# caburu/gym-supplychain

Hardware: AMD Instinct MI355X
Metric: env-steps/sec at 65536 envs/GPU, beergame-v0; 1/2/4/8 MI355X (higher is better)
Workload: dtype int32; 1 GPU; beergame-v0 step() x 65536 envs/GPU (BASELINE configs[1]; configs[4] at N=8); n_envs_per_gpu=65536, levels=4, weeks=35, auto_reset=True, ledgers=True, orders_history=True, episode_return_allgather=False, parallelism=env-shard x1

## Files before the change

### gym-supplychain_amd/csrc/scg_beergame.hip

```cpp

#include <cstdarg>
#include <cstdio>
#include <ctime>
#include <vector>

#include "scg_beergame_kernels.h"

namespace scg {

__global__ __launch_bounds__(kBlock) void poisson_demand_kernel(const BgArgs a, int32_t weeks,
                                                                int32_t* __restrict__ out) {
  const int64_t n = static_cast<int64_t>(blockIdx.x) * kBlock + threadIdx.x;
  if (n >= a.n) return;
  for (int32_t w = 1; w <= weeks; ++w) out[(int64_t)(w - 1) * a.n + n] = week_demand(a, n, w, a.episode);
}

__global__ __launch_bounds__(kBlock) void uniform_ints_kernel(uint32_t k0, uint32_t k1, int64_t env_offset,
                                                              int64_t n_envs, int32_t rows, int32_t width,
                                                              uint32_t tag, int32_t lo, uint32_t range,
                                                              int32_t* __restrict__ out) {
  const int64_t n = static_cast<int64_t>(blockIdx.x) * kBlock + threadIdx.x;
  if (n >= n_envs) return;
  const uint32_t env = static_cast<uint32_t>(env_offset + n);
  const int32_t words = rows * width;
  for (int32_t j0 = 0; j0 < words; j0 += 4) {
    const scg::U4 r = scg::philox4x32_10(scg::U4{env, tag, static_cast<uint32_t>(j0 >> 2), SCG_STREAM_ACTION}, k0, k1);
    const uint32_t w4[4] = {r.x, r.y, r.z, r.w};
#pragma unroll
    for (int s = 0; s < 4; ++s) {
      const int32_t j = j0 + s;
      if (j < words) {
        const uint32_t v = static_cast<uint32_t>((static_cast<uint64_t>(w4[s]) * range) >> 32);
        const int32_t rrow = j / width, col = j - rrow * width;
        out[((int64_t)rrow * n_envs + n) * width + col] = lo + static_cast<int32_t>(v);
      }
    }
  }
}

int launch_reset(int L, dim3 grid, hipStream_t s, const BgArgs& a) {
  switch (L) {
#define X(l) case l: return bg_launch_reset<l>(grid, s, a);
    SCG_LEVEL_CASES(X)
#undef X
    default: return fail(SCG_ERR_INVALID, "levels=%d outside 1..%d", L, SCG_BG_MAX_LEVELS);
  }
}

int launch_step2(int L, dim3 grid, hipStream_t s, const BgArgs& a, const WeekInfo& wk) {
  switch (L) {
#define X(l) case l: return bg_launch_step2<l>(grid, s, a, wk);
    SCG_LEVEL_CASES(X)
#undef X
    default: return fail(SCG_ERR_INVALID, "levels=%d outside 1..%d", L, SCG_BG_MAX_LEVELS);
  }
}

int launch_step(int L, dim3 grid, hipStream_t s, const BgArgs& a, const WeekInfo& wk, hipEvent_t ev0,
                hipEvent_t ev1) {
  switch (L) {
#define X(l) case l: return bg_launch_step<l>(grid, s, a, wk, ev0, ev1);
    SCG_LEVEL_CASES(X)
#undef X
    default: return fail(SCG_ERR_INVALID, "levels=%d outside 1..%d", L, SCG_BG_MAX_LEVELS);
  }
}

int launch_server(int L, int demand_mode, hipStream_t s, scg_bg_server_box* box, uint32_t exit_seen,
                  uint32_t idle_ticks) {
  switch (L) {
#define X(l) case l: return bg_launch_server<l>(s, demand_mode, box, exit_seen, idle_ticks);
    SCG_LEVEL_CASES(X)
#undef X
    default: return fail(SCG_ERR_INVALID, "levels=%d outside 1..%d", L, SCG_BG_MAX_LEVELS);
  }
}

int launch_slab(int demand_mode, int L, dim3 grid, hipStream_t s, int32_t* slab, const int32_t* act, int32_t* out,
                uint32_t n32, uint32_t wpack, uint32_t week, uint32_t episode, uint32_t k0, uint32_t k1,
                const BgSlabArgs& a, hipEvent_t ev0, hipEvent_t ev1) {
  switch (L) {
#define X(l) case l: return bg_launch_slab<l>(demand_mode, grid, s, slab, act, out, n32, wpack, week, episode, k0, k1, a, ev0, ev1);
    SCG_LEVEL_CASES(X)
#undef X
    default: return fail(SCG_ERR_INVALID, "levels=%d outside 1..%d", L, SCG_BG_MAX_LEVELS);
  }
}

int launch_rollout(int L, dim3 grid, hipStream_t s, const BgArgs& a, int32_t K, const RolloutWeeks& weeks,
                   const int32_t* acts, int32_t* obs, int32_t* rew) {
  switch (L) {
#define X(l) case l: return bg_launch_rollout<l>(grid, s, a, K, weeks, acts, obs, rew);
    SCG_LEVEL_CASES(X)
#undef X
    default: return fail(SCG_ERR_INVALID, "levels=%d outside 1..%d", L, SCG_BG_MAX_LEVELS);
  }
}

int slab_layout(int L, int64_t N, int32_t R, int32_t T, bool history, int64_t* off) {
  const int64_t NL = N * L;
  if (NL % 4 != 0) return fail(SCG_ERR_INVALID, "slab layout needs n_envs * levels %% 4 == 0 (got %lld)", (long long)NL);
  if (R < 1 || R > 127) return fail(SCG_ERR_INVALID, "slab layout needs 1 <= ring_slots <= 127");
  off[SCG_SLAB_ERROR] = 0;
  for (int f = 0; f < 6; ++f) off[SCG_SLAB_INVENTORY + f] = kSlabHeader + f * NL;
  off[SCG_SLAB_RING] = kSlabHeader + 6 * NL;
  off[SCG_SLAB_EPISODE_RETURN] = kSlabHeader + (6 + R) * NL;
  off[SCG_SLAB_FINAL_RETURN] = off[SCG_SLAB_EPISODE_RETURN] + 2 * N;
  off[SCG_SLAB_HISTORY] = off[SCG_SLAB_FINAL_RETURN] + 2 * N;
  off[SCG_SLAB_TOTAL] = off[SCG_SLAB_HISTORY] + (history ? static_cast<int64_t>(T + 1) * NL : 0);
  return SCG_OK;
}

bool slab_ready(const scg_bg_config* cfg, const scg_bg_state* st, const int32_t* obs, const int32_t* reward,
                const int32_t* terminal_obs) {
  if (!st->slab || cfg->variant != 1) return false;
  int64_t off[SCG_SLAB_FIELDS];
  const bool hist = st->orders_history != nullptr;
  if (slab_layout(cfg->levels, st->n_envs, cfg->ring_slots, cfg->max_weeks, hist, off) != SCG_OK) return false;
  int32_t* b = st->slab;
  const bool ledgers = st->inventory_costs != nullptr, returns = st->episode_return != nullptr;
  return st->inventory == b + off[SCG_SLAB_INVENTORY] && st->backlog == b + off[SCG_SLAB_BACKLOG] &&
         st->orders_placed == b + off[SCG_SLAB_ORDERS] && st->shipments == b + off[SCG_SLAB_RING] &&
         (!ledgers || (st->inventory_costs == b + off[SCG_SLAB_INV_COSTS] &&
                       st->backlog_costs == b + off[SCG_SLAB_BACKLOG_COSTS])) &&
         ledgers == (st->backlog_costs != nullptr) &&
         (!returns || (reinterpret_cast<int32_t*>(st->episode_return) == b + off[SCG_SLAB_EPISODE_RETURN] &&
                       reinterpret_cast<int32_t*>(st->final_return) == b + off[SCG_SLAB_FINAL_RETURN])) &&
         (!hist || st->orders_history == b + off[SCG_SLAB_HISTORY]) &&
         st->error_flags == b + off[SCG_SLAB_ERROR] && reward == obs + st->n_envs * cfg->levels &&
         (!terminal_obs || terminal_obs == b + off[SCG_SLAB_TERMINAL_OBS]);
}

int check_state(const scg_bg_config* cfg, const scg_bg_state* st) {
  if (!cfg || !st) return fail(SCG_ERR_INVALID, "null config/state");
  if (!cfg->plan || cfg->ring_slots <= 0) return fail(SCG_ERR_INVALID, "config not prepared (call scg_bg_prepare)");
  if (st->n_envs <= 0) return fail(SCG_ERR_INVALID, "n_envs must be > 0");
  if (st->n_envs > INT32_MAX) return fail(SCG_ERR_INVALID, "n_envs must be <= %d per shard", INT32_MAX);
  if (st->env_offset < 0 || st->env_offset + st->n_envs > (int64_t(1) << 32))
    return fail(SCG_ERR_INVALID, "global env ids must fit in 32 bits");
  if (!st->inventory || !st->backlog || !st->orders_placed || !st->shipments)
    return fail(SCG_ERR_INVALID, "state buffers inventory/backlog/orders_placed/shipments are required");
  if (cfg->demand_mode == SCG_DEMAND_TABLE && !cfg->demand_table)
    return fail(SCG_ERR_INVALID, "TABLE demand mode needs demand_table");
  if (cfg->demand_mode == SCG_DEMAND_POISSON && !cfg->poisson_thresholds)
    return fail(SCG_ERR_INVALID, "POISSON demand mode needs poisson_thresholds");
  return SCG_OK;
}

inline int32_t init_slots(const scg_bg_config* cfg) {
  const int32_t d0 = cfg->shipment_delays ? cfg->shipment_delays[0] : 0;
  return cfg->full_table ? d0 : std::min(d0, cfg->max_weeks);
}

BgArgs make_args(const scg_bg_config* cfg, const scg_bg_state* st) {
  BgArgs a;
  std::memset(&a, 0, sizeof(a));
  a.inv = st->inventory;
  a.bk = st->backlog;
  a.op = st->orders_placed;
  a.ring = st->shipments;
  a.inv_acc = st->inventory_costs;
  a.bk_acc = st->backlog_costs;
  a.hist = st->orders_history;
  a.ep_ret = st->episode_return;
  a.final_ret = st->final_return;
// ... 96 lines not shown
    if (cfg->variant != 1) return fail(SCG_ERR_INVALID, "full_table is a BeerGameEnv (variant 1) option");
    int32_t last = T + 1;
    for (int32_t w = 0; w <= T; ++w) last = std::max(last, w + cfg->shipment_delays[w] + 1);
    R = last + 1;
  }
  std::vector<uint8_t> written(static_cast<size_t>(T) + SCG_BG_MAX_DELAY + 2, 0);
  for (int32_t t = 1; t <= init_slots(cfg); ++t) written[t] = 1;
  cfg->plan[0] = 0;
  for (int32_t w = 1; w <= T; ++w) {
    const int32_t d = cfg->shipment_delays[w];
    int32_t mode;
    if (d == 0) {
      mode = MODE_DIRECT;
    } else if (w + d > T && !full) {
      mode = MODE_DROP;
    } else if (written[w + d]) {
      mode = MODE_ADD;
    } else {
      mode = MODE_STORE;
      written[w + d] = 1;
    }
    cfg->plan[w] = mode | (written[w] ? PLAN_ARRIVE : 0) | (d << 8);
  }
  cfg->ring_slots = R;
  return SCG_OK;
}

int scg_bg_slab_layout(const scg_bg_config* cfg, int64_t n_envs, int32_t with_history,
                       int64_t offsets[SCG_SLAB_FIELDS]) {
  if (!cfg || !offsets) return fail(SCG_ERR_INVALID, "null config/offsets");
  if (cfg->ring_slots <= 0) return fail(SCG_ERR_INVALID, "config not prepared (call scg_bg_prepare)");
  if (n_envs <= 0 || n_envs > INT32_MAX) return fail(SCG_ERR_INVALID, "n_envs must be in 1..%d", INT32_MAX);
  return slab_layout(cfg->levels, n_envs, cfg->ring_slots, cfg->max_weeks, with_history != 0, offsets);
}

int scg_bg_reset(const scg_bg_config* cfg, scg_bg_state* st, int32_t* obs, void* stream) {
  if (int rc = check_state(cfg, st)) return rc;
  if (st->week >= 0) st->episode += 1;
  BgArgs a = make_args(cfg, st);
  a.obs = obs;
  if (int rc = launch_reset(cfg->levels, grid_for(st->n_envs), static_cast<hipStream_t>(stream), a)) return rc;
  st->week = 0;
  return SCG_OK;
}

static scg::WeekInfo week_info(const scg_bg_config* cfg, int32_t w, uint32_t flags) {
  const int32_t p = cfg->plan[w];
  const int32_t R = cfg->ring_slots;
  WeekInfo wk;
  wk.week = w;
  wk.read_slot = plan_arrive(p) ? w % R : -1;
  wk.write_slot = (w + plan_delay(p)) % R;
  wk.mode = plan_mode(p);
  wk.demand_fixed = cfg->demand_mode == SCG_DEMAND_FIXED ? cfg->customer_demand[w - 1] : 0;
  const bool terminal = (w == cfg->max_weeks);
  wk.flags = (terminal ? 1 : 0) | ((terminal && (flags & SCG_BG_AUTORESET)) ? 2 : 0);
  return wk;
}

static int check_step(const scg_bg_config* cfg, const scg_bg_state* st) {
  if (st->week < 0) return fail(SCG_ERR_NOT_RESET, "step() before reset()");
  if (st->week >= cfg->max_weeks)
    return fail(SCG_ERR_PAST_HORIZON, "step() after the terminal week %d (customer_demand has %d weeks)",
                cfg->max_weeks, cfg->max_weeks);
  return SCG_OK;
}

int scg_bg_step(const scg_bg_config* cfg, scg_bg_state* st, const int32_t* action, int32_t* obs,
                int32_t* reward, int32_t* terminal_obs, uint32_t flags, int32_t* done, void* stream) {
  return scg_bg_step_timed(cfg, st, action, obs, reward, terminal_obs, flags, done, nullptr, nullptr, stream);
}

int scg_bg_step_timed(const scg_bg_config* cfg, scg_bg_state* st, const int32_t* action, int32_t* obs,
                      int32_t* reward, int32_t* terminal_obs, uint32_t flags, int32_t* done, void* start_event,
                      void* stop_event, void* stream) {
  if (int rc = check_state(cfg, st)) return rc;
  if (!action || !obs || !reward) return fail(SCG_ERR_INVALID, "action/obs/reward buffers are required");
  if (int rc = check_step(cfg, st)) return rc;
  const int32_t w = st->week + 1;
  const WeekInfo wk = week_info(cfg, w, flags);
  if (slab_ready(cfg, st, obs, reward, terminal_obs)) {
    BgSlabArgs sa;
    std::memset(&sa, 0, sizeof(sa));
    sa.pthr = cfg->poisson_thresholds;
    sa.demand_table = cfg->demand_table;
    sa.pthr_len = cfg->poisson_len;
    sa.h = cfg->inv_cost;
    sa.b = cfg->backlog_cost;
    sa.demand_fixed = wk.demand_fixed;
    sa.demand_lo = cfg->demand_lo;
    sa.demand_hi = cfg->demand_hi;
    sa.ship_value = cfg->initial_shipment_value;
    sa.orders_value = cfg->initial_orders_value;
    sa.init_slots = init_slots(cfg);
    sa.env_offset = st->env_offset;
    sa.guard = week_guard(cfg->levels, cfg->inv_cost, cfg->backlog_cost);
    sa.err_host = st->error_host;
    for (int l = 0; l < cfg->levels; ++l) sa.init_inv[l] = cfg->initial_inventory[l];
    uint32_t wpack = pack_week_slab(wk);
    wpack |= (wk.flags & 1) ? SW_TERMINAL : 0u;
    wpack |= (wk.flags & 2) ? SW_AUTORESET : 0u;
    wpack |= st->inventory_costs ? SW_LEDGERS : 0u;
    wpack |= st->episode_return ? SW_RETURNS : 0u;
    wpack |= st->orders_history ? SW_HISTORY : 0u;
    wpack |= static_cast<uint32_t>(cfg->ring_slots) << 24;
    if (int rc = launch_slab(cfg->demand_mode, cfg->levels, grid_for(st->n_envs), static_cast<hipStream_t>(stream),
                             st->slab, action, obs, static_cast<uint32_t>(st->n_envs), wpack, static_cast<uint32_t>(w),
                             st->episode, static_cast<uint32_t>(st->seed & 0xffffffffu),
                             static_cast<uint32_t>(st->seed >> 32), sa, static_cast<hipEvent_t>(start_event),
                             static_cast<hipEvent_t>(stop_event)))
      return rc;
    if (wk.flags & 2) {
      st->week = 0;
      st->episode += 1;
    } else {
      st->week = w;
    }
    if (done) *done = (wk.flags & 1) ? 1 : 0;
    return SCG_OK;
  }
  BgArgs a = make_args(cfg, st);
  a.act = action;
  a.obs = obs;
  a.rew = reward;
  a.term_obs = terminal_obs;
  if (cfg->variant == 2) {
    if (int rc = launch_step2(cfg->levels, grid_for(st->n_envs), static_cast<hipStream_t>(stream), a, wk)) return rc;
  } else if (int rc = launch_step(cfg->levels, grid_for(st->n_envs), static_cast<hipStream_t>(stream), a, wk,
                                  static_cast<hipEvent_t>(start_event), static_cast<hipEvent_t>(stop_event))) {
    return rc;
  }
  if (wk.flags & 2) {
    st->week = 0;
    st->episode += 1;
  } else {
    st->week = w;
  }
  if (done) *done = (wk.flags & 1) ? 1 : 0;
  return SCG_OK;
}

static_assert(sizeof(scg_bg_server_line) == 64, "request line");
static_assert(sizeof(scg_bg_server_box) == 17 * 64 + 64 + SCG_BG_SERVER_SLOTS * SCG_BG_SERVER_ARGS_BYTES, "mailbox");
static_assert(offsetof(scg_bg_server_box, done_seq) == 16 * 64 && offsetof(scg_bg_server_box, args) == 18 * 64,
              "mailbox lines");
static_assert(sizeof(scg_bg_server) == 72 && sizeof(scg_bg_server_slot) == 64, "server structs");
struct ServerLock {
  int32_t* w;
  explicit ServerLock(scg_bg_server* sv) : w(&sv->lock) {
    for (;;) {
      int32_t z = 0;
      if (__atomic_compare_exchange_n(w, &z, 1, false, __ATOMIC_ACQUIRE, __ATOMIC_RELAXED)) return;
      cpu_relax();
    }
  }
  ~ServerLock() { __atomic_store_n(w, 0, __ATOMIC_RELEASE); }
};

static bool server_ok(const scg_bg_server* sv) { return sv && sv->box_host && sv->box_dev; }

static int server_launch_locked(scg_bg_server* sv) {
  const uint32_t exit_seen = __atomic_load_n(&sv->box_host->exit_req, __ATOMIC_ACQUIRE);
  const uint32_t idle_ticks = static_cast<uint32_t>(sv->idle_us) * 100u;
  if (int rc = launch_server(sv->levels, sv->demand_mode, static_cast<hipStream_t>(sv->stream), sv->box_dev,
                             exit_seen, idle_ticks))
    return rc;
  sv->running = 1;
  sv->launches += 1;
  sv->last_ns = mono_ns();
  return SCG_OK;
}

static int server_stop_locked(scg_bg_server* sv) {
  if (!sv->running) return SCG_OK;
  __atomic_store_n(&sv->box_host->exit_req, sv->box_host->exit_req + 1, __ATOMIC_RELEASE);
  sv->running = 0;
  if (hipStreamSynchronize(static_cast<hipStream_t>(sv->stream)) != hipSuccess)
    return fail(SCG_ERR_HIP, "step server: hipStreamSynchronize failed");
  return SCG_OK;
}

int scg_bg_server_stop(scg_bg_server* sv) {
  if (!server_ok(sv)) return fail(SCG_ERR_INVALID, "null server/mailbox");
  ServerLock lk(sv);
  return server_stop_locked(sv);
}

uint32_t scg_bg_server_line_check(const scg_bg_server_line* line) {
  uint32_t w[16];
  std::memcpy(w, line, sizeof(w));
  return server_line_check(w);
}

// ... 212 lines not shown
```

### gym-supplychain_amd/csrc/scg_beergame_kernels.h

```cpp
#pragma once

#include <hip/hip_ext.h>
#include <hip/hip_runtime.h>

#include <algorithm>
#include <cmath>
#include <cstdint>
#include <cstdlib>
#include <cstring>

#include "scg_common.h"
#include "scg_mailbox.h"
#include "scg_const.h"
#include "scg_philox.h"
#include "scgpu.h"

namespace scg {

enum : int32_t { MODE_DIRECT = 0, MODE_STORE = 1, MODE_ADD = 2, MODE_DROP = 3 };
constexpr int32_t PLAN_ARRIVE = 4;
inline int32_t plan_mode(int32_t p) { return p & 3; }
inline bool plan_arrive(int32_t p) { return (p & PLAN_ARRIVE) != 0; }
inline int32_t plan_delay(int32_t p) { return (p >> 8) & 0xff; }

constexpr int kBlock = 256;

struct BgArgs {
  int32_t* inv;
  int32_t* bk;
  int32_t* op;
  int32_t* ring;
  int32_t* inv_acc;
  int32_t* bk_acc;
  int32_t* hist;
  int64_t* ep_ret;
  int64_t* final_ret;
  const int32_t* act;
  int32_t* obs;
  int32_t* rew;
  int32_t* term_obs;
  const int32_t* demand_table;
  const uint32_t* pthr;
  int64_t n;
  int64_t env_offset;
  uint32_t key0, key1;
  uint32_t episode;
  int32_t demand_mode;
  int32_t pthr_len;
  int32_t h, b;
  int32_t ship_value, orders_value;
  int32_t init_slots;
  int32_t ring_slots;
  int32_t init_inv[SCG_BG_MAX_LEVELS];
  int32_t* pen_acc;
  int32_t max_stock, penalty;
  int32_t demand_lo, demand_hi;
  int32_t stochastic_delays, delay_lo, delay_hi, max_weeks;
  int32_t* err;
  int32_t guard;
  int32_t* err_host;
};

#ifndef SCG_BG_OVERFLOW_CHECK
#define SCG_BG_OVERFLOW_CHECK 1
#endif
__device__ __forceinline__ bool fits32(int64_t x) {
  return !SCG_BG_OVERFLOW_CHECK || x == static_cast<int64_t>(static_cast<int32_t>(x));
}
__device__ __forceinline__ int out32(int64_t x) { return fits32(x) ? 0 : 1; }

__device__ __forceinline__ void note_overflow(int32_t* err, bool ovf) {
  if (ovf && err) *reinterpret_cast<volatile int32_t*>(err) = 1;
}

__device__ __forceinline__ void export_error(int64_t n, bool terminal, const int32_t* err, int32_t* err_host) {
  if (terminal && n == 0 && err && err_host)
    *reinterpret_cast<volatile int32_t*>(err_host) = *reinterpret_cast<const volatile int32_t*>(err);
}

template <int L>
__device__ __forceinline__ void load_row(const int32_t* __restrict__ p, int32_t (&v)[L]) {
  if constexpr (L % 4 == 0) {
#pragma unroll
    for (int c = 0; c < L / 4; ++c) {
      const int4 t = reinterpret_cast<const int4*>(p)[c];
      v[4 * c] = t.x; v[4 * c + 1] = t.y; v[4 * c + 2] = t.z; v[4 * c + 3] = t.w;
    }
  } else if constexpr (L % 2 == 0) {
#pragma unroll
// ... 386 lines not shown
static_assert(sizeof(BgArgs) <= SCG_BG_SERVER_ARGS_BYTES, "BgArgs outgrew the mailbox's argument blocks");
static_assert(kServerSlots <= 16 && kServerArgWords <= 2 * kServerBlock, "server layout");

template <int L, int DM>
__global__ __launch_bounds__(kServerBlock) void bg_server_kernel(scg_bg_server_box* box, uint32_t exit_seen,
                                                                 uint32_t idle_ticks) {
  __shared__ __align__(16) uint32_t s_args[kServerSlots][kServerArgWords];
  __shared__ uint32_t s_last[16], s_gen[16];
  const int lane = threadIdx.x;
  if (lane < 16) {
    s_last[lane] = __hip_atomic_load(&box->done_seq[lane], __ATOMIC_RELAXED, __HIP_MEMORY_SCOPE_SYSTEM);
    s_gen[lane] = 0;
  }
  __syncthreads();
  const uint32_t* lines = reinterpret_cast<const uint32_t*>(box->req);
  uint64_t t0 = __builtin_amdgcn_s_memrealtime();
  uint32_t ex = exit_seen;
  uint32_t ns = __hip_atomic_load(&box->n_slots, __ATOMIC_RELAXED, __HIP_MEMORY_SCOPE_SYSTEM);
  for (;;) {
    const int n_slots = __builtin_amdgcn_readfirstlane(static_cast<int>(ns < kServerSlots ? ns : kServerSlots));
    ns = __hip_atomic_load(&box->n_slots, __ATOMIC_RELAXED, __HIP_MEMORY_SCOPE_SYSTEM);
    ex = __hip_atomic_load(&box->exit_req, __ATOMIC_RELAXED, __HIP_MEMORY_SCOPE_SYSTEM);
    uint32_t v[4] = {0, 0, 0, 0};
#pragma unroll
    for (int r = 0; r < 4; ++r) {
      const int slot = 4 * r + (lane >> 4);
      if (slot < n_slots)
        v[r] = __hip_atomic_load(lines + slot * 16 + (lane & 15), __ATOMIC_RELAXED, __HIP_MEMORY_SCOPE_SYSTEM);
    }
    bool served = false;
    for (int slot = 0; slot < n_slots; ++slot) {
      const int base = (slot & 3) * 16, r = slot >> 2;
      const uint32_t vr = r == 0 ? v[0] : r == 1 ? v[1] : r == 2 ? v[2] : v[3];
      const uint32_t seq = __builtin_amdgcn_readlane(vr, base);
      if (seq == s_last[slot]) continue;
      uint32_t w[16];
#pragma unroll
      for (int i = 0; i < 16; ++i) w[i] = __builtin_amdgcn_readlane(vr, base + i);
      if (w[7] != server_line_check(w)) continue;
      __builtin_amdgcn_fence(__ATOMIC_ACQUIRE, "");
      if (w[6] != s_gen[slot]) {
        const uint32_t* src = reinterpret_cast<const uint32_t*>(box->args[slot]);
        for (int k = lane; k < kServerArgWords; k += kServerBlock)
          s_args[slot][k] = __hip_atomic_load(src + k, __ATOMIC_RELAXED, __HIP_MEMORY_SCOPE_SYSTEM);
        __syncthreads();
        if (lane == 0) s_gen[slot] = w[6];
      }
      const BgArgs& a = *reinterpret_cast<const BgArgs*>(s_args[slot]);
      WeekInfo wk{};
      wk.week = static_cast<int32_t>(w[3]);
      wk.demand_fixed = static_cast<int32_t>(w[4]);
      const int64_t n = lane;
      if (n < a.n) {
        if (L <= 8 && static_cast<int32_t>(w[5]) == L) {
          int32_t act_in[L];
#pragma unroll
          for (int l = 0; l < L; ++l) act_in[l] = static_cast<int32_t>(w[8 + (l < 8 ? l : 0)]);
          bg_step_env<L, DM, true>(n, a.inv, a.bk, a.op, a.act, a.ring, static_cast<uint32_t>(a.n), w[2], a, wk, act_in);
        } else {
          bg_step_env<L, DM>(n, a.inv, a.bk, a.op, a.act, a.ring, static_cast<uint32_t>(a.n), w[2], a, wk);
        }
      }
      __builtin_amdgcn_fence(__ATOMIC_RELEASE, "");
      if (lane == 0) {
        __hip_atomic_store(&box->done_seq[slot], seq, __ATOMIC_RELEASE, __HIP_MEMORY_SCOPE_SYSTEM);
        s_last[slot] = seq;
      }
      __syncthreads();
      served = true;
    }
    if (ex != exit_seen) break;
    if (served) {
      t0 = __builtin_amdgcn_s_memrealtime();
      continue;
    }
    if (__builtin_amdgcn_s_memrealtime() - t0 > idle_ticks) break;
    __builtin_amdgcn_s_sleep(2);
  }
  __builtin_amdgcn_fence(__ATOMIC_RELEASE, "");
  if (lane == 0) __hip_atomic_store(&box->exit_seq, ex, __ATOMIC_RELEASE, __HIP_MEMORY_SCOPE_SYSTEM);
}

struct BgSlabArgs {
  const uint32_t* pthr;
  const int32_t* demand_table;
  int32_t pthr_len;
  int32_t h, b;
  int32_t demand_fixed;
  int32_t demand_lo, demand_hi;
  int32_t ship_value, orders_value, init_slots;
  int64_t env_offset;
  int32_t guard;
  int32_t* err_host;
  int32_t init_inv[SCG_BG_MAX_LEVELS];
};


constexpr uint32_t SW_TERMINAL = 1u << 18, SW_AUTORESET = 1u << 19, SW_LEDGERS = 1u << 20, SW_RETURNS = 1u << 21,
                   SW_HISTORY = 1u << 22;
constexpr int kSlabHeader = 4;

template <int L, int DM>
__global__ __launch_bounds__(kBlock) void bg_step_slab_kernel(int32_t* __restrict__ slab, const int32_t* __restrict__ act_p,
                                                              int32_t* __restrict__ out, uint32_t n32, uint32_t wpack,
                                                              uint32_t week, uint32_t episode, uint32_t key0,
                                                              uint32_t key1, const BgSlabArgs a) {
  const int64_t n = static_cast<int64_t>(blockIdx.x) * kBlock + threadIdx.x;
  if (n >= static_cast<int64_t>(n32)) return;
  const int32_t read_slot = static_cast<int32_t>(wpack & 0xffu) - 1;
  const int32_t write_slot = static_cast<int32_t>((wpack >> 8) & 0xffu);
  const int32_t mode = static_cast<int32_t>((wpack >> 16) & 3u);
  const int32_t R = static_cast<int32_t>((wpack >> 24) & 0x7fu);
  const bool terminal = wpack & SW_TERMINAL, autoreset = wpack & SW_AUTORESET;
  const bool ledgers = wpack & SW_LEDGERS, returns = wpack & SW_RETURNS, history = wpack & SW_HISTORY;
  const int64_t NL = static_cast<int64_t>(n32) * L;
  const int64_t row = n * L;
  int32_t* const rows = slab + kSlabHeader;
  int32_t* const inv_p = rows, *const bk_p = rows + NL, *const op_p = rows + 2 * NL;
  int32_t* const iacc_p = rows + 3 * NL, *const bacc_p = rows + 4 * NL, *const term_p = rows + 5 * NL;
  int32_t* const ring_p = rows + 6 * NL;
  int64_t* const ret_p = reinterpret_cast<int64_t*>(rows + (6 + R) * NL);
  int64_t* const fret_p = ret_p + n32;
  int32_t* const hist_p = reinterpret_cast<int32_t*>(fret_p + n32);

  int32_t inv[L], bk[L], op[L], act[L], due[L], cur[L], iacc[L], bacc[L];
  zero_row<L>(due);
  zero_row<L>(cur);
  zero_row<L>(iacc);
  zero_row<L>(bacc);
  load_row<L>(inv_p + row, inv);
  load_row<L>(bk_p + row, bk);
  load_row<L>(op_p + row, op);
  load_row<L>(act_p + row, act);
  if (read_slot >= 0) load_row<L>(ring_p + read_slot * NL + row, due);
  if (mode == MODE_ADD) load_row<L>(ring_p + write_slot * NL + row, cur);
  if (ledgers && !autoreset) {
    load_row<L>(iacc_p + row, iacc);
    load_row<L>(bacc_p + row, bacc);
  }
  const int64_t ret0 = returns ? ret_p[n] : 0;
  export_error(n, terminal, slab, a.err_host);
  int32_t demand;
  if constexpr (DM == SCG_DEMAND_FIXED) {
    demand = a.demand_fixed;
  } else if constexpr (DM == SCG_DEMAND_TABLE) {
    demand = a.demand_table[static_cast<int64_t>(week - 1) * n32 + n];
  } else if constexpr (DM == SCG_DEMAND_UNIFORM) {
    const uint32_t w = scg::philox_word(key0, key1, static_cast<uint32_t>(a.env_offset + n), episode, week - 1,
                                        SCG_STREAM_BG2_DEMAND);
    demand = a.demand_lo + static_cast<int32_t>((static_cast<uint64_t>(w) * static_cast<uint32_t>(a.demand_hi - a.demand_lo)) >> 32);
  } else {
    const uint32_t u = scg::philox_word(key0, key1, static_cast<uint32_t>(a.env_offset + n), episode, week - 1,
                                        SCG_STREAM_DEMAND);
    demand = poisson_count_scalar(const_tab(a.pthr), a.pthr_len, u);
  }

  int32_t ship[L], obs[L];
  bool ovf = false;
  const int32_t reward = week_update<L>(a.h, a.b, a.guard, demand, mode == MODE_DIRECT, due, inv, bk, op, act, ship,
                                        obs, cur, iacc, bacc, ovf);
  if (mode == MODE_STORE) {
    store_row_p<L>(ring_p + write_slot * NL + row, ship);
  } else if (mode == MODE_ADD) {
    store_row_p<L>(ring_p + write_slot * NL + row, cur);
  }
  out[NL + n] = reward;
  if (history) store_row_p<L>(hist_p + static_cast<int64_t>(week) * NL + row, op);
  const int64_t ret = ret0 + reward;
  if (terminal) {
    store_row_p<L>(term_p + row, obs);
    if (returns) fret_p[n] = ret;
  }
  if (autoreset) {
    int32_t v[L];
#pragma unroll
    for (int l = 0; l < L; ++l) v[l] = a.init_inv[l];
    store_row_p<L>(inv_p + row, v);
    store_row_p<L>(out + row, v);
    fill_row_p<L>(bk_p + row, 0);
    fill_row_p<L>(op_p + row, a.orders_value);
    for (int t = 1; t <= a.init_slots; ++t) fill_row_p<L>(ring_p + (t % R) * NL + row, a.ship_value);
    if (ledgers) {
      fill_row_p<L>(iacc_p + row, 0);
      fill_row_p<L>(bacc_p + row, 0);
    }
    if (history) fill_row_p<L>(hist_p + row, a.orders_value);
    if (returns) ret_p[n] = 0;
    note_overflow(slab, ovf);
    return;
  }
  store_row_p<L>(inv_p + row, inv);
  store_row_p<L>(bk_p + row, bk);
  store_row_p<L>(op_p + row, op);
  store_row_p<L>(out + row, obs);
  if (ledgers) {
    store_row_p<L>(iacc_p + row, iacc);
    store_row_p<L>(bacc_p + row, bacc);
  }
  if (returns) ret_p[n] = ret;
  note_overflow(slab, ovf);
}

template <int L>
__global__ __launch_bounds__(kBlock) void bg2_step_kernel(const BgArgs a, const WeekInfo wk) {
  const int64_t n = static_cast<int64_t>(blockIdx.x) * kBlock + threadIdx.x;
  if (n >= a.n) return;
  const int64_t row = n * L;
  const int64_t stride = a.n * L;
  const bool terminal = wk.flags & 1;
  const bool autoreset = wk.flags & 2;
  int32_t read_slot = wk.read_slot, write_slot = wk.write_slot, mode = wk.mode;
  if (a.stochastic_delays) {
    const uint32_t u = scg::philox_word(a.key0, a.key1, static_cast<uint32_t>(a.env_offset + n), a.episode,
                                        static_cast<uint32_t>(wk.week - 1), SCG_STREAM_BG2_DELAY);
    const int32_t d = a.delay_lo + static_cast<int32_t>((static_cast<uint64_t>(u) * static_cast<uint32_t>(a.delay_hi - a.delay_lo)) >> 32);
    read_slot = wk.week % a.ring_slots;
    write_slot = (wk.week + d) % a.ring_slots;
    mode = d == 0 ? MODE_DIRECT : (wk.week + d > a.max_weeks ? MODE_DROP : MODE_ADD);
  }
  int32_t inv[L], bk[L], op[L], act[L], due[L], cur[L], iacc[L], bacc[L], pacc[L];
  load_row<L>(a.inv + row, inv);
  load_row<L>(a.bk + row, bk);
  load_row<L>(a.op + row, op);
  load_row<L>(a.act + row, act);
  zero_row<L>(due);
  zero_row<L>(cur);
  zero_row<L>(iacc);
  zero_row<L>(bacc);
  zero_row<L>(pacc);
  if (read_slot >= 0) load_row<L>(a.ring + read_slot * stride + row, due);
  if (mode == MODE_ADD) load_row<L>(a.ring + write_slot * stride + row, cur);
  if (!autoreset && a.inv_acc) load_row<L>(a.inv_acc + row, iacc);
  if (!autoreset && a.bk_acc) load_row<L>(a.bk_acc + row, bacc);
  if (!autoreset && a.pen_acc) load_row<L>(a.pen_acc + row, pacc);
  const int64_t ret0 = a.ep_ret ? a.ep_ret[n] : 0;
  export_error(n, terminal, a.err, a.err_host);
  const int32_t demand = a.demand_mode == SCG_DEMAND_FIXED ? wk.demand_fixed : week_demand(a, n, wk.week, a.episode);

  int64_t inc[L], iv[L], fill[L], del[L], sh[L];
  int32_t ship[L], obs[L];
  bool ovf = false;
  inc[0] = demand;
// ... 127 lines not shown
    if (a.demand_mode == SCG_DEMAND_FIXED)
      demand = wk.demand_fixed;
    else
      demand = week_demand(a, n, wk.week, episode);
    zero_row<L>(cur);
    if (wk.mode == MODE_ADD) ring.load(wk.write_slot, cur);
    const int32_t reward = week_update<L>(a.h, a.b, a.guard, demand, wk.mode == MODE_DIRECT, due, inv, bk, op, act, ship,
                                          obs, cur, iacc, bacc, ovf);
    if (wk.mode == MODE_STORE) {
      ring.store(wk.write_slot, ship);
    } else if (wk.mode == MODE_ADD) {
      ring.store(wk.write_slot, cur);
    }
    if (a.hist) store_row<L>(a.hist + static_cast<int64_t>(wk.week) * stride + row, op);
    ret += reward;
    if ((wk.flags & 1) && a.final_ret) a.final_ret[n] = ret;
    if (wk.flags & 2) {
#pragma unroll
      for (int l = 0; l < L; ++l) {
        inv[l] = a.init_inv[l];
        bk[l] = 0;
        op[l] = a.orders_value;
        iacc[l] = bacc[l] = 0;
        obs[l] = inv[l];
      }
      int32_t init[L];
#pragma unroll
      for (int l = 0; l < L; ++l) init[l] = a.ship_value;
      for (int t = 1; t <= a.init_slots; ++t) ring.store(t % a.ring_slots, init);
      if (a.hist) fill_row<L>(a.hist + row, a.orders_value);
      ret = 0;
      ++episode;
    }
    if (obs_out) store_row<L>(obs_out + k * stride + row, obs);
    if (rew_out) rew_out[k * a.n + n] = reward;
  }
  }
  store_row<L>(a.inv + row, inv);
  store_row<L>(a.bk + row, bk);
  store_row<L>(a.op + row, op);
  if (a.inv_acc) store_row<L>(a.inv_acc + row, iacc);
  if (a.bk_acc) store_row<L>(a.bk_acc + row, bacc);
  if (a.ep_ret) a.ep_ret[n] = ret;
  note_overflow(a.err, ovf);
}

template <int L>
__global__ __launch_bounds__(kBlock) void bg_rollout_kernel(const BgArgs a, int32_t K, const RolloutWeeks weeks,
                                                            const int32_t* __restrict__ acts, int32_t* __restrict__ obs_out,
                                                            int32_t* __restrict__ rew_out) {
  const int64_t n = static_cast<int64_t>(blockIdx.x) * kBlock + threadIdx.x;
  if (n >= a.n) return;
  rollout_body<L>(a, n, K, weeks, acts, obs_out, rew_out, RingHbm<L>{a.ring, a.n * L, n * L});
}

template <int L>
__global__ __launch_bounds__(kBlock) void bg_rollout_lds_kernel(const BgArgs a, int32_t K, const RolloutWeeks weeks,
                                                                const int32_t* __restrict__ acts,
                                                                int32_t* __restrict__ obs_out,
                                                                int32_t* __restrict__ rew_out) {
  extern __shared__ int32_t lds_ring[];
  const int64_t n = static_cast<int64_t>(blockIdx.x) * kBlock + threadIdx.x;
  if (n >= a.n) return;
  const RingHbm<L> hbm{a.ring, a.n * L, n * L};
  const RingLds<L> lds{lds_ring + threadIdx.x};
  for (int s = 0; s < a.ring_slots; ++s) {
    int32_t v[L];
    hbm.load(s, v);
    lds.store(s, v);
  }
  rollout_body<L>(a, n, K, weeks, acts, obs_out, rew_out, lds);
  for (int s = 0; s < a.ring_slots; ++s) {
    int32_t v[L];
    lds.load(s, v);
    hbm.store(s, v);
  }
}

#ifndef SCG_MODULE_LAUNCH
#define SCG_MODULE_LAUNCH 1
#endif

template <int L, int DM>
int launch_slab_module(dim3 grid, hipStream_t s, int32_t* slab, const int32_t* act, int32_t* out, uint32_t n32,
                       uint32_t wpack, uint32_t week, uint32_t episode, uint32_t k0, uint32_t k1, const BgSlabArgs& a) {
  static hipFunction_t fn = nullptr;
  if (!fn && hipGetFuncBySymbol(&fn, reinterpret_cast<const void*>(&bg_step_slab_kernel<L, DM>)) != hipSuccess)
    return fail(SCG_ERR_HIP, "hipGetFuncBySymbol(bg_step_slab_kernel) failed");
  BgSlabArgs args = a;
  void* params[] = {&slab, &act, &out, &n32, &wpack, &week, &episode, &k0, &k1, &args};
  if (hipModuleLaunchKernel(fn, grid.x, 1, 1, kBlock, 1, 1, 0, s, params, nullptr) != hipSuccess)
    return fail(SCG_ERR_HIP, "hipModuleLaunchKernel(bg_step_slab_kernel) failed");
  return SCG_OK;
}

template <int L>
int bg_launch_reset(dim3 grid, hipStream_t s, const BgArgs& a) {
  hipLaunchKernelGGL(bg_reset_kernel<L>, grid, dim3(kBlock), 0, s, a);
  return check_launch("bg_reset_kernel");
}

template <int L>
int bg_launch_step2(dim3 grid, hipStream_t s, const BgArgs& a, const WeekInfo& wk) {
  hipLaunchKernelGGL(bg2_step_kernel<L>, grid, dim3(kBlock), 0, s, a, wk);
  return check_launch("bg2_step_kernel");
}

template <int L, int DM>
int bg_launch_step_dm(dim3 grid, hipStream_t s, const BgArgs& a, const WeekInfo& wk, hipEvent_t ev0, hipEvent_t ev1) {
  hipExtLaunchKernelGGL(HIP_KERNEL_NAME(bg_step_kernel<L, DM>), grid, dim3(kBlock), 0, s, ev0, ev1, 0, a.inv, a.bk, a.op,
                        a.act, a.ring, static_cast<uint32_t>(a.n), pack_week(wk), a, wk);
  return check_launch("bg_step_kernel");
}

template <int L>
int bg_launch_step(dim3 grid, hipStream_t s, const BgArgs& a, const WeekInfo& wk, hipEvent_t ev0, hipEvent_t ev1) {
  switch (a.demand_mode) {
    case SCG_DEMAND_FIXED: return bg_launch_step_dm<L, SCG_DEMAND_FIXED>(grid, s, a, wk, ev0, ev1);
    case SCG_DEMAND_TABLE: return bg_launch_step_dm<L, SCG_DEMAND_TABLE>(grid, s, a, wk, ev0, ev1);
    case SCG_DEMAND_UNIFORM: return bg_launch_step_dm<L, SCG_DEMAND_UNIFORM>(grid, s, a, wk, ev0, ev1);
    default: return bg_launch_step_dm<L, SCG_DEMAND_POISSON>(grid, s, a, wk, ev0, ev1);
  }
}

template <int L>
int bg_launch_server(hipStream_t s, int demand_mode, scg_bg_server_box* box, uint32_t exit_seen, uint32_t idle_ticks) {
  switch (demand_mode) {
    case SCG_DEMAND_FIXED:
      hipLaunchKernelGGL(HIP_KERNEL_NAME(bg_server_kernel<L, SCG_DEMAND_FIXED>), dim3(1), dim3(kServerBlock), 0, s, box,
                         exit_seen, idle_ticks);
      break;
    case SCG_DEMAND_TABLE:
      hipLaunchKernelGGL(HIP_KERNEL_NAME(bg_server_kernel<L, SCG_DEMAND_TABLE>), dim3(1), dim3(kServerBlock), 0, s, box,
                         exit_seen, idle_ticks);
      break;
    case SCG_DEMAND_UNIFORM:
      hipLaunchKernelGGL(HIP_KERNEL_NAME(bg_server_kernel<L, SCG_DEMAND_UNIFORM>), dim3(1), dim3(kServerBlock), 0, s, box,
                         exit_seen, idle_ticks);
      break;
    default:
      hipLaunchKernelGGL(HIP_KERNEL_NAME(bg_server_kernel<L, SCG_DEMAND_POISSON>), dim3(1), dim3(kServerBlock), 0, s, box,
                         exit_seen, idle_ticks);
  }
  return check_launch("bg_server_kernel");
}

template <int L, int DM>
int bg_launch_slab_dm(dim3 grid, hipStream_t s, int32_t* slab, const int32_t* act, int32_t* out, uint32_t n32,
                      uint32_t wpack, uint32_t week, uint32_t episode, uint32_t k0, uint32_t k1, const BgSlabArgs& a,
                      hipEvent_t ev0, hipEvent_t ev1) {
  if (ev0 || ev1) {
    hipExtLaunchKernelGGL(HIP_KERNEL_NAME(bg_step_slab_kernel<L, DM>), grid, dim3(kBlock), 0, s, ev0, ev1, 0, slab, act,
                          out, n32, wpack, week, episode, k0, k1, a);
    return check_launch("bg_step_slab_kernel");
  }
  if (SCG_MODULE_LAUNCH) return launch_slab_module<L, DM>(grid, s, slab, act, out, n32, wpack, week, episode, k0, k1, a);
  hipLaunchKernelGGL(HIP_KERNEL_NAME(bg_step_slab_kernel<L, DM>), grid, dim3(kBlock), 0, s, slab, act, out, n32, wpack,
                     week, episode, k0, k1, a);
  return check_launch("bg_step_slab_kernel");
}

template <int L>
int bg_launch_slab(int demand_mode, dim3 grid, hipStream_t s, int32_t* slab, const int32_t* act, int32_t* out,
                   uint32_t n32, uint32_t wpack, uint32_t week, uint32_t episode, uint32_t k0, uint32_t k1,
                   const BgSlabArgs& a, hipEvent_t ev0, hipEvent_t ev1) {
  switch (demand_mode) {
    case SCG_DEMAND_FIXED:
      return bg_launch_slab_dm<L, SCG_DEMAND_FIXED>(grid, s, slab, act, out, n32, wpack, week, episode, k0, k1, a, ev0, ev1);
    case SCG_DEMAND_TABLE:
      return bg_launch_slab_dm<L, SCG_DEMAND_TABLE>(grid, s, slab, act, out, n32, wpack, week, episode, k0, k1, a, ev0, ev1);
    case SCG_DEMAND_UNIFORM:
      return bg_launch_slab_dm<L, SCG_DEMAND_UNIFORM>(grid, s, slab, act, out, n32, wpack, week, episode, k0, k1, a, ev0,
                                                      ev1);
    default:
      return bg_launch_slab_dm<L, SCG_DEMAND_POISSON>(grid, s, slab, act, out, n32, wpack, week, episode, k0, k1, a, ev0,
                                                      ev1);
  }
}

template <int L>
int bg_launch_rollout(dim3 grid, hipStream_t s, const BgArgs& a, int32_t K, const RolloutWeeks& weeks,
                      const int32_t* acts, int32_t* obs, int32_t* rew) {
  const size_t lds = static_cast<size_t>(a.ring_slots) * L * kBlock * sizeof(int32_t);
  if (lds <= 64 * 1024) {
    hipLaunchKernelGGL(bg_rollout_lds_kernel<L>, grid, dim3(kBlock), lds, s, a, K, weeks, acts, obs, rew);
    return check_launch("bg_rollout_lds_kernel");
  }
  hipLaunchKernelGGL(bg_rollout_kernel<L>, grid, dim3(kBlock), 0, s, a, K, weeks, acts, obs, rew);
  return check_launch("bg_rollout_kernel");
}

#define SCG_LEVEL_CASES(X) X(1) X(2) X(3) X(4) X(5) X(6) X(7) X(8) X(9) X(10) X(11) X(12) X(13) X(14) X(15) X(16)

#define SCG_BG_LAUNCHERS(EXT, l)                                                                                     \
  EXT template int bg_launch_reset<l>(dim3, hipStream_t, const BgArgs&);                                            \
  EXT template int bg_launch_step2<l>(dim3, hipStream_t, const BgArgs&, const WeekInfo&);                           \
  EXT template int bg_launch_step<l>(dim3, hipStream_t, const BgArgs&, const WeekInfo&, hipEvent_t, hipEvent_t);    \
  EXT template int bg_launch_server<l>(hipStream_t, int, scg_bg_server_box*, uint32_t, uint32_t);                   \
  EXT template int bg_launch_slab<l>(int, dim3, hipStream_t, int32_t*, const int32_t*, int32_t*, uint32_t, uint32_t, \
                                     uint32_t, uint32_t, uint32_t, uint32_t, const BgSlabArgs&, hipEvent_t,         \
                                     hipEvent_t);                                                                    \
  EXT template int bg_launch_rollout<l>(dim3, hipStream_t, const BgArgs&, int32_t, const RolloutWeeks&,             \
                                        const int32_t*, int32_t*, int32_t*);
#define SCG_BG_EXTERN_LEVEL(l) SCG_BG_LAUNCHERS(extern, l)
SCG_LEVEL_CASES(SCG_BG_EXTERN_LEVEL)
#undef SCG_BG_EXTERN_LEVEL

}
```

Baseline: 13.71 billion env-steps/s.

## Batch slab kernel scalar loads and preload Poisson thresholds into SGPRs

Reorders the slab kernel arguments so the out pointer, costs, guard and demand parameters can be fetched with one aligned s_load_dwordx8 from the kernarg segment. For Poisson demand, the first 32 threshold entries are prefetched into SGPRs with two s_load_dwordx16 before the slab loads, and the Philox draw is issued before a single lgkmcnt wait, so scalar latency overlaps with vector work. Error export is now done only on terminal steps, and the week and table length are packed into one argument. This relies on a hard-coded kernarg offset and inline asm, which is fragile if the argument layout or the compiler's kernarg handling changes.

```diff
diff --git a/gym-supplychain_amd/csrc/scg_beergame.hip b/gym-supplychain_amd/csrc/scg_beergame.hip
--- a/gym-supplychain_amd/csrc/scg_beergame.hip
+++ b/gym-supplychain_amd/csrc/scg_beergame.hip
@@ -76,11 +76,11 @@
   }
 }
 
-int launch_slab(int demand_mode, int L, dim3 grid, hipStream_t s, int32_t* slab, const int32_t* act, int32_t* out,
-                uint32_t n32, uint32_t wpack, uint32_t week, uint32_t episode, uint32_t k0, uint32_t k1,
+int launch_slab(int demand_mode, int L, dim3 grid, hipStream_t s, int32_t* slab, const int32_t* act, const void* dsrc,
+                uint32_t n32, uint32_t wpack, uint32_t wlen, uint32_t episode, uint64_t key, int64_t env_offset,
                 const BgSlabArgs& a, hipEvent_t ev0, hipEvent_t ev1) {
   switch (L) {
-#define X(l) case l: return bg_launch_slab<l>(demand_mode, grid, s, slab, act, out, n32, wpack, week, episode, k0, k1, a, ev0, ev1);
+#define X(l) case l: return bg_launch_slab<l>(demand_mode, grid, s, slab, act, dsrc, n32, wpack, wlen, episode, key, env_offset, a, ev0, ev1);
     SCG_LEVEL_CASES(X)
 #undef X
     default: return fail(SCG_ERR_INVALID, "levels=%d outside 1..%d", L, SCG_BG_MAX_LEVELS);
@@ -343,21 +343,26 @@
   if (slab_ready(cfg, st, obs, reward, terminal_obs)) {
     BgSlabArgs sa;
     std::memset(&sa, 0, sizeof(sa));
-    sa.pthr = cfg->poisson_thresholds;
-    sa.demand_table = cfg->demand_table;
-    sa.pthr_len = cfg->poisson_len;
+    sa.err_host = st->error_host;
+    sa.out = obs;
     sa.h = cfg->inv_cost;
     sa.b = cfg->backlog_cost;
+    sa.guard = week_guard(cfg->levels, cfg->inv_cost, cfg->backlog_cost);
     sa.demand_fixed = wk.demand_fixed;
     sa.demand_lo = cfg->demand_lo;
     sa.demand_hi = cfg->demand_hi;
     sa.ship_value = cfg->initial_shipment_value;
     sa.orders_value = cfg->initial_orders_value;
     sa.init_slots = init_slots(cfg);
-    sa.env_offset = st->env_offset;
-    sa.guard = week_guard(cfg->levels, cfg->inv_cost, cfg->backlog_cost);
-    sa.err_host = st->error_host;
     for (int l = 0; l < cfg->levels; ++l) sa.init_inv[l] = cfg->initial_inventory[l];
+    const void* dsrc = nullptr;
+    int32_t pthr_len = 0;
+    if (cfg->demand_mode == SCG_DEMAND_POISSON) {
+      dsrc = cfg->poisson_thresholds;
+      pthr_len = cfg->poisson_len;
+    } else if (cfg->demand_mode == SCG_DEMAND_TABLE) {
+      dsrc = cfg->demand_table;
+    }
     uint32_t wpack = pack_week_slab(wk);
     wpack |= (wk.flags & 1) ? SW_TERMINAL : 0u;
     wpack |= (wk.flags & 2) ? SW_AUTORESET : 0u;
@@ -366,10 +371,9 @@
     wpack |= st->orders_history ? SW_HISTORY : 0u;
     wpack |= static_cast<uint32_t>(cfg->ring_slots) << 24;
     if (int rc = launch_slab(cfg->demand_mode, cfg->levels, grid_for(st->n_envs), static_cast<hipStream_t>(stream),
-                             st->slab, action, obs, static_cast<uint32_t>(st->n_envs), wpack, static_cast<uint32_t>(w),
-                             st->episode, static_cast<uint32_t>(st->seed & 0xffffffffu),
-                             static_cast<uint32_t>(st->seed >> 32), sa, static_cast<hipEvent_t>(start_event),
-                             static_cast<hipEvent_t>(stop_event)))
+                             st->slab, action, dsrc, static_cast<uint32_t>(st->n_envs), wpack, pack_week_len(w, pthr_len),
+                             st->episode, static_cast<uint64_t>(st->seed), st->env_offset, sa,
+                             static_cast<hipEvent_t>(start_event), static_cast<hipEvent_t>(stop_event)))
       return rc;
     if (wk.flags & 2) {
       st->week = 0;
diff --git a/gym-supplychain_amd/csrc/scg_beergame_kernels.h b/gym-supplychain_amd/csrc/scg_beergame_kernels.h
--- a/gym-supplychain_amd/csrc/scg_beergame_kernels.h
+++ b/gym-supplychain_amd/csrc/scg_beergame_kernels.h
@@ -5,6 +5,7 @@
 
 #include <algorithm>
 #include <cmath>
+#include <cstddef>
 #include <cstdint>
 #include <cstdlib>
 #include <cstring>
@@ -557,19 +558,66 @@
 }
 
 struct BgSlabArgs {
-  const uint32_t* pthr;
-  const int32_t* demand_table;
-  int32_t pthr_len;
-  int32_t h, b;
+  int32_t* err_host;
+  int32_t* out;
+  int32_t h, b, guard;
   int32_t demand_fixed;
   int32_t demand_lo, demand_hi;
   int32_t ship_value, orders_value, init_slots;
-  int64_t env_offset;
-  int32_t guard;
-  int32_t* err_host;
   int32_t init_inv[SCG_BG_MAX_LEVELS];
 };
-
+constexpr int kSlabArgsOffset = 56;
+constexpr int kSlabBatchOffset = kSlabArgsOffset + 8;
+static_assert(offsetof(BgSlabArgs, out) == 8 && offsetof(BgSlabArgs, h) == 16 && offsetof(BgSlabArgs, b) == 20 &&
+                  offsetof(BgSlabArgs, guard) == 24 && offsetof(BgSlabArgs, demand_fixed) == 28 &&
+                  offsetof(BgSlabArgs, demand_lo) == 32 && offsetof(BgSlabArgs, demand_hi) == 36 &&
+                  alignof(BgSlabArgs) == 8 && kSlabBatchOffset % 64 == 0,
+              "the slab kernel reads BgSlabArgs::out .. demand_hi as one aligned 8-dword batch");
+
+static_assert(SCG_BG_MAX_WEEKS < (1 << 16) && SCG_POISSON_MAX < (1 << 16), "week / table length field too narrow");
+inline uint32_t pack_week_len(int32_t week, int32_t pthr_len) {
+  return static_cast<uint32_t>(week) | (static_cast<uint32_t>(pthr_len) << 16);
+}
+
+typedef uint32_t u32x8 __attribute__((ext_vector_type(8)));
+typedef uint32_t u32x16 __attribute__((ext_vector_type(16)));
+constexpr int kPoissonBatch = 32;
+
+__device__ __forceinline__ int32_t count16(u32x16 t, uint32_t u) {
+  int32_t x = 0;
+#pragma unroll
+  for (int j = 0; j < 16; ++j) x += (t[j] <= u) ? 1 : 0;
+  return x;
+}
+
+__device__ __forceinline__ u32x16 load16_clamped(ConstTab<uint32_t> thr, int32_t k0, int32_t len) {
+  u32x16 t;
+#pragma unroll
+  for (int j = 0; j < 16; ++j) t[j] = thr[min(k0 + j, len - 1)];
+  return t;
+}
+
+__device__ __forceinline__ int32_t count_clamped_excess(uint32_t last_row, int32_t rows, int32_t have, uint32_t u) {
+  return last_row <= u ? rows - have : 0;
+}
+
+__device__ __forceinline__ int32_t poisson_count_rest(ConstTab<uint32_t> thr, int32_t k0, int32_t len, uint32_t u) {
+  int32_t x = 0;
+  int k = k0;
+  for (; k + 8 <= len; k += 8) {
+#pragma unroll
+    for (int j = 0; j < 8; ++j) x += (thr[k + j] <= u) ? 1 : 0;
+  }
+  if (k < len) {
+    uint32_t t[7];
+#pragma unroll
+    for (int j = 0; j < 7; ++j) t[j] = thr[min(k + j, len - 1)];
+#pragma unroll
+    for (int j = 0; j < 7; ++j) x += (t[j] <= u) ? 1 : 0;
+    x -= count_clamped_excess(t[6], 7, len - k, u);
+  }
+  return x;
+}
 
 constexpr uint32_t SW_TERMINAL = 1u << 18, SW_AUTORESET = 1u << 19, SW_LEDGERS = 1u << 20, SW_RETURNS = 1u << 21,
                    SW_HISTORY = 1u << 22;
@@ -577,11 +625,26 @@
 
 template <int L, int DM>
 __global__ __launch_bounds__(kBlock) void bg_step_slab_kernel(int32_t* __restrict__ slab, const int32_t* __restrict__ act_p,
-                                                              int32_t* __restrict__ out, uint32_t n32, uint32_t wpack,
-                                                              uint32_t week, uint32_t episode, uint32_t key0,
-                                                              uint32_t key1, const BgSlabArgs a) {
+                                                              const void* __restrict__ dsrc, uint32_t n32, uint32_t wpack,
+                                                              uint32_t wlen, uint32_t episode, uint64_t key,
+                                                              int64_t env_offset, const BgSlabArgs a) {
   const int64_t n = static_cast<int64_t>(blockIdx.x) * kBlock + threadIdx.x;
   if (n >= static_cast<int64_t>(n32)) return;
+  const uint32_t week = wlen & 0xffffu;
+  const int32_t pthr_len = static_cast<int32_t>(wlen >> 16);
+  const ConstTab<uint32_t> thr = const_tab(static_cast<const uint32_t*>(dsrc));
+  u32x16 thr0 = {}, thr1 = {};
+  const bool thr_whole = pthr_len >= kPoissonBatch;
+  if constexpr (DM == SCG_DEMAND_POISSON) {
+    if (thr_whole) {
+      asm volatile("s_load_dwordx16 %0, %2, 0x0\n\ts_load_dwordx16 %1, %2, 0x40" : "=&s"(thr0), "=&s"(thr1) : "s"(thr));
+    } else {
+      thr0 = load16_clamped(thr, 0, pthr_len);
+      thr1 = load16_clamped(thr, 16, pthr_len);
+    }
+  }
+  u32x8 batch;
+  asm volatile("s_load_dwordx8 %0, %1, %2" : "=s"(batch) : "s"(__builtin_amdgcn_kernarg_segment_ptr()), "i"(kSlabBatchOffset));
   const int32_t read_slot = static_cast<int32_t>(wpack & 0xffu) - 1;
   const int32_t write_slot = static_cast<int32_t>((wpack >> 8) & 0xffu);
   const int32_t mode = static_cast<int32_t>((wpack >> 16) & 3u);
@@ -614,25 +677,47 @@
     load_row<L>(bacc_p + row, bacc);
   }
   const int64_t ret0 = returns ? ret_p[n] : 0;
-  export_error(n, terminal, slab, a.err_host);
+  int32_t table_demand = 0;
+  if constexpr (DM == SCG_DEMAND_TABLE)
+    table_demand = static_cast<const int32_t*>(dsrc)[static_cast<int64_t>(week - 1) * n32 + n];
+  if (terminal) export_error(n, true, slab, a.err_host);
+  const uint32_t key0 = static_cast<uint32_t>(key), key1 = static_cast<uint32_t>(key >> 32);
+  uint32_t u = 0;
+  if constexpr (DM == SCG_DEMAND_UNIFORM) {
+    u = scg::philox_word(key0, key1, static_cast<uint32_t>(env_offset + n), episode, week - 1, SCG_STREAM_BG2_DEMAND);
+  } else if constexpr (DM == SCG_DEMAND_POISSON) {
+    u = scg::philox_word(key0, key1, static_cast<uint32_t>(env_offset + n), episode, week - 1, SCG_STREAM_DEMAND);
+  }
+  if constexpr (DM == SCG_DEMAND_POISSON) {
+    asm volatile("s_waitcnt lgkmcnt(0)" : "+s"(batch), "+s"(thr0), "+s"(thr1), "+v"(u));
+  } else if constexpr (DM == SCG_DEMAND_UNIFORM) {
+    asm volatile("s_waitcnt lgkmcnt(0)" : "+s"(batch), "+v"(u));
+  } else {
+    asm volatile("s_waitcnt lgkmcnt(0)" : "+s"(batch));
+  }
+  int32_t* const out = reinterpret_cast<int32_t*>(static_cast<uint64_t>(batch[0]) | (static_cast<uint64_t>(batch[1]) << 32));
+  const int32_t h = static_cast<int32_t>(batch[2]), b = static_cast<int32_t>(batch[3]);
+  const int32_t guard = static_cast<int32_t>(batch[4]);
   int32_t demand;
   if constexpr (DM == SCG_DEMAND_FIXED) {
-    demand = a.demand_fixed;
+    demand = static_cast<int32_t>(batch[5]);
   } else if constexpr (DM == SCG_DEMAND_TABLE) {
-    demand = a.demand_table[static_cast<int64_t>(week - 1) * n32 + n];
+    demand = table_demand;
   } else if constexpr (DM == SCG_DEMAND_UNIFORM) {
-    const uint32_t w = scg::philox_word(key0, key1, static_cast<uint32_t>(a.env_offset + n), episode, week - 1,
-                                        SCG_STREAM_BG2_DEMAND);
-    demand = a.demand_lo + static_cast<int32_t>((static_cast<uint64_t>(w) * static_cast<uint32_t>(a.demand_hi - a.demand_lo)) >> 32);
+    const int32_t lo = static_cast<int32_t>(batch[6]), hi = static_cast<int32_t>(batch[7]);
+    demand = lo + static_cast<int32_t>((static_cast<uint64_t>(u) * static_cast<uint32_t>(hi - lo)) >> 32);
   } else {
-    const uint32_t u = scg::philox_word(key0, key1, static_cast<uint32_t>(a.env_offset + n), episode, week - 1,
-                                        SCG_STREAM_DEMAND);
-    demand = poisson_count_scalar(const_tab(a.pthr), a.pthr_len, u);
+    demand = count16(thr0, u) + count16(thr1, u);
+    if (thr_whole) {
+      demand += poisson_count_rest(thr, kPoissonBatch, pthr_len, u);
+    } else {
+      demand -= count_clamped_excess(thr1[15], kPoissonBatch, pthr_len, u);
+    }
   }
 
   int32_t ship[L], obs[L];
   bool ovf = false;
-  const int32_t reward = week_update<L>(a.h, a.b, a.guard, demand, mode == MODE_DIRECT, due, inv, bk, op, act, ship,
+  const int32_t reward = week_update<L>(h, b, guard, demand, mode == MODE_DIRECT, due, inv, bk, op, act, ship,
                                         obs, cur, iacc, bacc, ovf);
   if (mode == MODE_STORE) {
     store_row_p<L>(ring_p + write_slot * NL + row, ship);
@@ -926,13 +1011,14 @@
 #endif
 
 template <int L, int DM>
-int launch_slab_module(dim3 grid, hipStream_t s, int32_t* slab, const int32_t* act, int32_t* out, uint32_t n32,
-                       uint32_t wpack, uint32_t week, uint32_t episode, uint32_t k0, uint32_t k1, const BgSlabArgs& a) {
+int launch_slab_module(dim3 grid, hipStream_t s, int32_t* slab, const int32_t* act, const void* dsrc, uint32_t n32,
+                       uint32_t wpack, uint32_t wlen, uint32_t episode, uint64_t key, int64_t env_offset,
+                       const BgSlabArgs& a) {
   static hipFunction_t fn = nullptr;
   if (!fn && hipGetFuncBySymbol(&fn, reinterpret_cast<const void*>(&bg_step_slab_kernel<L, DM>)) != hipSuccess)
     return fail(SCG_ERR_HIP, "hipGetFuncBySymbol(bg_step_slab_kernel) failed");
   BgSlabArgs args = a;
-  void* params[] = {&slab, &act, &out, &n32, &wpack, &week, &episode, &k0, &k1, &args};
+  void* params[] = {&slab, &act, &dsrc, &n32, &wpack, &wlen, &episode, &key, &env_offset, &args};
   if (hipModuleLaunchKernel(fn, grid.x, 1, 1, kBlock, 1, 1, 0, s, params, nullptr) != hipSuccess)
     return fail(SCG_ERR_HIP, "hipModuleLaunchKernel(bg_step_slab_kernel) failed");
   return SCG_OK;
@@ -990,35 +1076,38 @@
 }
 
 template <int L, int DM>
-int bg_launch_slab_dm(dim3 grid, hipStream_t s, int32_t* slab, const int32_t* act, int32_t* out, uint32_t n32,
-                      uint32_t wpack, uint32_t week, uint32_t episode, uint32_t k0, uint32_t k1, const BgSlabArgs& a,
-                      hipEvent_t ev0, hipEvent_t ev1) {
+int bg_launch_slab_dm(dim3 grid, hipStream_t s, int32_t* slab, const int32_t* act, const void* dsrc, uint32_t n32,
+                      uint32_t wpack, uint32_t wlen, uint32_t episode, uint64_t key, int64_t env_offset,
+                      const BgSlabArgs& a, hipEvent_t ev0, hipEvent_t ev1) {
   if (ev0 || ev1) {
     hipExtLaunchKernelGGL(HIP_KERNEL_NAME(bg_step_slab_kernel<L, DM>), grid, dim3(kBlock), 0, s, ev0, ev1, 0, slab, act,
-                          out, n32, wpack, week, episode, k0, k1, a);
+                          dsrc, n32, wpack, wlen, episode, key, env_offset, a);
     return check_launch("bg_step_slab_kernel");
   }
-  if (SCG_MODULE_LAUNCH) return launch_slab_module<L, DM>(grid, s, slab, act, out, n32, wpack, week, episode, k0, k1, a);
-  hipLaunchKernelGGL(HIP_KERNEL_NAME(bg_step_slab_kernel<L, DM>), grid, dim3(kBlock), 0, s, slab, act, out, n32, wpack,
-                     week, episode, k0, k1, a);
+  if (SCG_MODULE_LAUNCH)
+    return launch_slab_module<L, DM>(grid, s, slab, act, dsrc, n32, wpack, wlen, episode, key, env_offset, a);
+  hipLaunchKernelGGL(HIP_KERNEL_NAME(bg_step_slab_kernel<L, DM>), grid, dim3(kBlock), 0, s, slab, act, dsrc, n32, wpack,
+                     wlen, episode, key, env_offset, a);
   return check_launch("bg_step_slab_kernel");
 }
 
 template <int L>
-int bg_launch_slab(int demand_mode, dim3 grid, hipStream_t s, int32_t* slab, const int32_t* act, int32_t* out,
-                   uint32_t n32, uint32_t wpack, uint32_t week, uint32_t episode, uint32_t k0, uint32_t k1,
+int bg_launch_slab(int demand_mode, dim3 grid, hipStream_t s, int32_t* slab, const int32_t* act, const void* dsrc,
+                   uint32_t n32, uint32_t wpack, uint32_t wlen, uint32_t episode, uint64_t key, int64_t env_offset,
                    const BgSlabArgs& a, hipEvent_t ev0, hipEvent_t ev1) {
   switch (demand_mode) {
     case SCG_DEMAND_FIXED:
-      return bg_launch_slab_dm<L, SCG_DEMAND_FIXED>(grid, s, slab, act, out, n32, wpack, week, episode, k0, k1, a, ev0, ev1);
+      return bg_launch_slab_dm<L, SCG_DEMAND_FIXED>(grid, s, slab, act, dsrc, n32, wpack, wlen, episode, key, env_offset, a,
+                                                    ev0, ev1);
     case SCG_DEMAND_TABLE:
-      return bg_launch_slab_dm<L, SCG_DEMAND_TABLE>(grid, s, slab, act, out, n32, wpack, week, episode, k0, k1, a, ev0, ev1);
+      return bg_launch_slab_dm<L, SCG_DEMAND_TABLE>(grid, s, slab, act, dsrc, n32, wpack, wlen, episode, key, env_offset, a,
+                                                    ev0, ev1);
     case SCG_DEMAND_UNIFORM:
-      return bg_launch_slab_dm<L, SCG_DEMAND_UNIFORM>(grid, s, slab, act, out, n32, wpack, week, episode, k0, k1, a, ev0,
-                                                      ev1);
+      return bg_launch_slab_dm<L, SCG_DEMAND_UNIFORM>(grid, s, slab, act, dsrc, n32, wpack, wlen, episode, key, env_offset,
+                                                      a, ev0, ev1);
     default:
-      return bg_launch_slab_dm<L, SCG_DEMAND_POISSON>(grid, s, slab, act, out, n32, wpack, week, episode, k0, k1, a, ev0,
-                                                      ev1);
+      return bg_launch_slab_dm<L, SCG_DEMAND_POISSON>(grid, s, slab, act, dsrc, n32, wpack, wlen, episode, key, env_offset,
+                                                      a, ev0, ev1);
   }
 }
 
@@ -1041,8 +1130,8 @@
   EXT template int bg_launch_step2<l>(dim3, hipStream_t, const BgArgs&, const WeekInfo&);                           \
   EXT template int bg_launch_step<l>(dim3, hipStream_t, const BgArgs&, const WeekInfo&, hipEvent_t, hipEvent_t);    \
   EXT template int bg_launch_server<l>(hipStream_t, int, scg_bg_server_box*, uint32_t, uint32_t);                   \
-  EXT template int bg_launch_slab<l>(int, dim3, hipStream_t, int32_t*, const int32_t*, int32_t*, uint32_t, uint32_t, \
-                                     uint32_t, uint32_t, uint32_t, uint32_t, const BgSlabArgs&, hipEvent_t,         \
+  EXT template int bg_launch_slab<l>(int, dim3, hipStream_t, int32_t*, const int32_t*, const void*, uint32_t,       \
+                                     uint32_t, uint32_t, uint32_t, uint64_t, int64_t, const BgSlabArgs&, hipEvent_t, \
                                      hipEvent_t);                                                                    \
   EXT template int bg_launch_rollout<l>(dim3, hipStream_t, const BgArgs&, int32_t, const RolloutWeeks&,             \
                                         const int32_t*, int32_t*, int32_t*);
```

Measured after the change: 13.14 billion env-steps/s. 4.2% lower.
